# ChristianFeldmann/libHM

Measured on AMD Instinct MI355X. Metric: decoded Mpixels/s (luma), 2160p Main10 reconstruction + loop filters, higher is better.
Workload: dtype int16 samples / int32 accumulate; 1 GPU; 3840x2160 Main10 lowdelay_P pictures, pre-parsed CTU metadata: prep+MC+dequant/IT/recon+deblock+SAO, batch of 16 independent pictures per step, inputs resident in HBM; sub_benchmark=full, streams=2, parallelism=frame-parallel, 1 process per GPU, no data-path collective

## Files before the change

### libhm_amd/csrc/hmgpu_api.hip

```cpp
#include "hmgpu_host.h"

#include <algorithm>
#include <cstdio>
#include <cstring>
#include <cstdlib>
#include <new>
#include <vector>

namespace hmgpu_host __attribute__((visibility("hidden"))) {

hipError_t h2d_small(hmgpu_ctx* c, void* dst, const void* src, size_t bytes, hipStream_t hs) {
  const size_t need = (bytes + 63) & ~(size_t)63;
  if (!c->bounce || need > hmgpu_ctx::kBounceSeg) return hipMemcpyAsync(dst, src, bytes, hipMemcpyHostToDevice, hs);
  if (c->bounce_off + need > hmgpu_ctx::kBounceSeg) {
    hipStream_t streams[3] = {c->stream, c->copy_stream, c->copy_stream2};
    for (int k = 0; k < 3; k++) (void)hipEventRecord(c->bounce_ev[c->bounce_seg][k], streams[k]);
    c->bounce_used[c->bounce_seg] = true;
    c->bounce_seg = (c->bounce_seg + 1) % hmgpu_ctx::kBounceSegs;
    c->bounce_off = 0;
    if (c->bounce_used[c->bounce_seg]) for (int k = 0; k < 3; k++) (void)hipEventSynchronize(c->bounce_ev[c->bounce_seg][k]);
  }
  char* at = c->bounce + (size_t)c->bounce_seg * hmgpu_ctx::kBounceSeg + c->bounce_off;
  memcpy(at, src, bytes);
  c->bounce_off += need;
// ... 217 lines not shown

namespace hmgpu_host __attribute__((visibility("hidden"))) {

hmgpu_status run_recon(hmgpu_ctx* c, const Batch& b, bool any_intra, bool any_wp, bool any_cells, bool any_bi, bool any_islice) {
  int max_ctus = 0;
  for (int i = 0; i < b.n; i++) max_ctus = std::max(max_ctus, b.num_ctus[i]);
  { ProfScope ps(c, K_PREP); launch_prep(c->d_pics, b, max_ctus, c->parts, any_intra, any_bi, any_cells || c->fmt != 1, c->fmt, c->stream); }
  if (c->fmt != 1) {
    for (int i = 0; i < b.n; i++) {
      const PicDev& d = c->pics[b.pic[i]].dev;
      HIP_TRY(c, hipMemsetAsync(d.resid[1], 0, (size_t)((char*)d.resid[2] - (char*)d.resid[1]) + c->coef_elems[2] * sizeof(int16_t), c->stream));
    }
  }
  McArgs ma;
  memset(&ma, 0, sizeof(ma));
  ma.n = b.n; ma.width = c->seq.width; ma.height = c->seq.height; ma.log2ctu = c->seq.log2_ctu_size; ma.ctus_w = c->ctus_w;
  ma.tw = c->grid_w / 2; ma.npics = c->seq.max_pictures;
  ma.slab = c->plane_slab; ma.pic_stride = 2 * c->plane_bytes; ma.slab_bytes = ma.pic_stride * c->pics.size(); ma.sao_off = (uint32_t)c->plane_bytes;
  for (size_t i = 0; i < c->pics.size(); i++)
    if (c->pics[i].sao_applied) (i < 32 ? ma.sao_mask_lo : ma.sao_mask_hi) |= 1u << (i & 31);
  for (int i = 0; i < b.n; i++) {
    const PicDev& d = c->pics[b.pic[i]].dev;
    ma.first_ctu[i] = b.first_ctu[i]; ma.num_ctus[i] = b.num_ctus[i];
    ma.tmv[i] = d.tmv; ma.slices[i] = d.slices;
  }
  const PicDev& d0 = c->pics[b.pic[0]].dev;
  const char* const base0 = (const char*)c->pics[b.pic[0]].planes;
  uint32_t bps = (uint32_t)std::max(4, std::min(b.n >= 4 ? 12 : 24, max_ctus / 8 + 1));
  {
    ItxArgs ia;
    memset(&ia, 0, sizeof(ia));
    ia.n = b.n; ia.class_mask = 0xf;
    for (int k = 0; k < 3; k++) { ia.rtw[k] = (c->grid_w / 2) >> (k ? c->csx : 0); ia.bd[k] = d0.bd[k]; }
    ia.csx = c->csx; ia.csy = c->csy;
    for (int k = 0; k < 4; k++) ia.tu_cap[k] = c->tu_cap[k];
    for (int i = 0; i < b.n; i++) {
      const PicDev& d = c->pics[b.pic[i]].dev;
      for (int k = 0; k < 4; k++) ia.tu[i][k] = d.tu[k];
      ia.tu_count[i] = d.tu_count;
      for (int k = 0; k < 3; k++) { ia.coef[i][k] = d.coef[k]; ia.resid[i][k] = d.resid[k]; }
      ia.sl_m[i] = d.sl_m;
    }
    ProfScope ps(c, K_ITX);
    launch_itx(ia, bps, c->stream);
    bool any_ccp = false;
    for (int i = 0; i < b.n; i++) any_ccp |= c->pics[b.pic[i]].dev.ccp[0] != nullptr;
    if (any_ccp) launch_ccp(c->d_pics, b, max_ctus, c->stream);
  }
  {
    ProfScope ps(c, K_MC_LUMA);
    ma.pitch = c->pitch[0]; ma.bd = c->seq.bit_depth_luma;
    ma.origin_off = (uint32_t)((const char*)d0.rec[0] - base0);
    ma.rtw = c->grid_w / 2;
    for (int i = 0; i < b.n; i++) { ma.dst[i] = c->pics[b.pic[i]].dev.rec[0]; ma.resid[i] = c->pics[b.pic[i]].dev.resid[0]; }
    launch_mc_luma(ma, max_ctus, any_wp, any_bi, c->stream);
    if (any_cells) { ProfScope pc(c, K_MC_CELLS); launch_mc_luma_cells(c->d_pics, c->d_finals, b, max_ctus, c->seq.log2_ctu_size, any_wp, c->stream); }
  }
  if (c->fmt != 1) {
    ProfScope ps(c, K_MC_CHROMA);
    launch_mc_chroma_fmt(c->d_pics, c->d_finals, b, max_ctus, c->seq.log2_ctu_size, c->fmt, any_wp, c->stream);
  } else if (c->seq.chroma_format != 0) {
    ProfScope ps(c, K_MC_CHROMA);
    ma.pitch = c->pitch[1]; ma.bd = c->seq.bit_depth_chroma;
    ma.origin_off = (uint32_t)((const char*)d0.rec[1] - base0);
    ma.cr_off = 0;
    ma.rtw = c->grid_w / 4;
    for (int i = 0; i < b.n; i++) {
      const PicDev& d = c->pics[b.pic[i]].dev;
      ma.dst[i] = d.rec[1]; ma.dst2[i] = d.rec[2]; ma.resid[i] = d.resid[1]; ma.resid2[i] = d.resid[2];
    }
    launch_mc_chroma(ma, max_ctus, any_wp, any_bi, c->stream);
    if (any_cells) { ProfScope pc(c, K_MC_CELLS); launch_mc_chroma_cells(c->d_pics, c->d_finals, b, max_ctus, c->seq.log2_ctu_size, any_wp, c->stream); }
  }
  if (any_intra) {
    ProfScope ps(c, K_INTRA);
    launch_intra(c->d_pics, b, c->d_ctu_order, c->num_ctus, !any_islice, c->stream);
    if (c->fmt == 2) launch_intra_chroma_422(c->d_pics, b, c->stream);
    for (int i = 0; i < b.n; i++) if (std::find(c->intra_launched.begin(), c->intra_launched.end(), b.pic[i]) == c->intra_launched.end()) c->intra_launched.push_back(b.pic[i]);
  }
  HIP_TRY(c, hipGetLastError());
  return HMGPU_OK;
}

hmgpu_status run_filter(hmgpu_ctx* c, const Batch& b, int stages) {
  bool all_sao = stages == 7 && c->fmt == 1;
  for (int i = 0; i < b.n && all_sao; i++) all_sao = c->pics[b.pic[i]].sao_any;
  if (all_sao) {
    bool nofilt = false;
    for (int i = 0; i < b.n; i++) nofilt |= c->pics[b.pic[i]].dev.any_nofilt != 0;
    { ProfScope ps(c, K_FILTER); launch_filter_fused(c->d_pics, b, c->seq.width, c->seq.height, nofilt, c->stream); }
    HIP_TRY(c, hipGetLastError());
    return HMGPU_OK;
  }
  if (stages & 1) { ProfScope ps(c, K_DBK_VER); launch_deblock(c->d_pics, b, 0, c->seq.width, c->seq.height, c->stream);
                    if (c->fmt != 1) launch_deblock_chroma_fmt(c->d_pics, b, 0, c->seq.width, c->seq.height, c->stream); }
  if (stages & 2) { ProfScope ps(c, K_DBK_HOR); launch_deblock(c->d_pics, b, 1, c->seq.width, c->seq.height, c->stream);
                    if (c->fmt != 1) launch_deblock_chroma_fmt(c->d_pics, b, 1, c->seq.width, c->seq.height, c->stream); }
  if (stages & 4) {
    bool any = false;
    for (int i = 0; i < b.n; i++) any |= c->pics[b.pic[i]].sao_any;
    if (any) { ProfScope ps(c, K_SAO); launch_sao(c->d_pics, b, c->seq.width, c->seq.height, c->csx, c->csy, c->stream); }
  }
  HIP_TRY(c, hipGetLastError());
  return HMGPU_OK;
}

hmgpu_status stage_sao(hmgpu_ctx* c, Picture& p, const hmgpu_pic_params* pp, const hmgpu_sao_param* sao,
                       const std::vector<uint16_t>& slice_idx, const std::vector<uint16_t>& tile_idx) {
  const int n = c->num_ctus;
  std::vector<const hmgpu_sao_param*> res((size_t)n * 3);
  std::vector<SaoDev>& dev = p.h_saoprm;
  dev.resize((size_t)n * 3);
  bool any = false;
  for (int a = 0; a < n; a++) {
    const int cx = a % c->ctus_w, cy = a / c->ctus_w;
    const hmgpu_sao_param* const* merge[2] = {nullptr, nullptr};
    auto same = [&](int o) { return slice_idx[o] == slice_idx[a] && tile_idx[o] == tile_idx[a]; };
    if (cx > 0 && same(a - 1)) merge[HMGPU_SAO_MERGE_LEFT] = &res[(size_t)(a - 1) * 3];
    if (cy > 0 && same(a - c->ctus_w)) merge[HMGPU_SAO_MERGE_ABOVE] = &res[(size_t)(a - c->ctus_w) * 3];
    unsigned avail = 1u << 4;
    for (int k = 0; k < 9; k++) {
      if (k == 4) continue;
      const int nx = cx + k % 3 - 1, ny = cy + k / 3 - 1;
      if (nx < 0 || nx >= c->ctus_w || ny < 0 || ny >= c->ctus_h) continue;
      const int o = ny * c->ctus_w + nx;
      bool ok = true;
      if (slice_idx[o] != slice_idx[a]) {
        const SliceDev& later = p.slices[std::max(slice_idx[o], slice_idx[a])];
        ok = later.lf_across_slices != 0;
      }
      if (ok && !pp->lf_across_tiles) ok = tile_idx[o] == tile_idx[a];
      if (ok) avail |= 1u << k;
    }
    for (int comp = 0; comp < 3; comp++) {
      const hmgpu_sao_param* r = &sao[(size_t)a * 3 + comp];
      if (r->mode_idc == HMGPU_SAO_MERGE) {
        if (r->type_idc < 0 || r->type_idc > 1 || !merge[r->type_idc]) return HMGPU_EINVAL;
        r = merge[r->type_idc][comp];
      }
      res[(size_t)a * 3 + comp] = r;
      const int shift = comp == 0 ? pp->sao_offset_shift_luma : pp->sao_offset_shift_chroma;
      SaoDev& d = dev[(size_t)a * 3 + comp];
      memset(&d, 0, sizeof(d));
      d.type = r->mode_idc == HMGPU_SAO_OFF ? -1 : (int8_t)r->type_idc;
      d.avail = (uint16_t)avail;
      if (d.type == HMGPU_SAO_BO) {
        d.band = (uint8_t)(r->type_aux_info & 31);
        for (int i = 0; i < 4; i++) d.off[i] = (int8_t)(r->offset[(r->type_aux_info + i) & 31] * (1 << shift));
      } else if (d.type >= 0) {
        for (int i = 0; i < 5; i++) d.off[i] = (int8_t)(r->offset[i] * (1 << shift));
      }
      any |= d.type >= 0;
    }
  }
  p.sao_any = any;
  HIP_TRY(c, h2d_small(c, p.dev.saoprm, dev.data(), dev.size() * sizeof(SaoDev), c->stream));
  return HMGPU_OK;
}

}

extern "C" {

const char* hmgpu_status_string(hmgpu_status s) {
  switch (s) {
    case HMGPU_OK: return "ok";
    case HMGPU_EINVAL: return "invalid argument";
    case HMGPU_EDEVICE: return "device (HIP) error";
    case HMGPU_EUNSUPPORTED: return "coding tool not supported";
    case HMGPU_ENOMEM: return "out of memory";
  }
  return "?";
}
const char* hmgpu_kernel_name(int32_t k) { return (k >= 0 && k < HMGPU_NUM_KERNELS) ? kKernelNames[k] : ""; }
// ... 283 lines not shown
  if (p.sao_applied) return HMGPU_EINVAL;
  coverage_clear(p);
  p.extended = true;
  return HMGPU_OK;
}

hmgpu_status hmgpu_picture_transfer(hmgpu_ctx* src, hmgpu_pic src_pic, hmgpu_ctx* dst, hmgpu_pic dst_pic) {
  if (!src || !dst || !valid_pic(src, src_pic) || !valid_pic(dst, dst_pic) || (src == dst && src_pic == dst_pic)) return HMGPU_EINVAL;
  const hmgpu_seq_params &a = src->seq, &b = dst->seq;
  if (a.width != b.width || a.height != b.height || a.log2_ctu_size != b.log2_ctu_size || a.bit_depth_luma != b.bit_depth_luma ||
      a.bit_depth_chroma != b.bit_depth_chroma) return HMGPU_EINVAL;
  void *from = nullptr, *to = nullptr;
  int64_t n_from = 0, n_to = 0;
  hmgpu_status st = hmgpu_picture_device_region(src, src_pic, HMGPU_REGION_FINISHED, &from, &n_from);
  if (st == HMGPU_OK) st = hmgpu_picture_device_region(dst, dst_pic, HMGPU_REGION_RECEIVE, &to, &n_to);
  if (st != HMGPU_OK) return st;
  if (n_from != n_to) return HMGPU_EINVAL;
  if (src->device != dst->device) {
    int can = 0;
    if (hipDeviceCanAccessPeer(&can, dst->device, src->device) == hipSuccess && can) {
      hipSetDevice(dst->device);
      const hipError_t e = hipDeviceEnablePeerAccess(src->device, 0);
      if (e != hipSuccess && e != hipErrorPeerAccessAlreadyEnabled) return HMGPU_EDEVICE;
      (void)hipGetLastError();
    }
  }
  hipSetDevice(src->device);
  if (!src->xfer_ev[0]) for (int k = 0; k < 2; k++) HIP_TRY(src, hipEventCreateWithFlags(&src->xfer_ev[k], hipEventDisableTiming));
  HIP_TRY(src, hipEventRecord(src->xfer_ev[0], src->stream));
  hipSetDevice(dst->device);
  HIP_TRY(dst, hipStreamWaitEvent(dst->stream, src->xfer_ev[0], 0));
  HIP_TRY(dst, hipMemcpyPeerAsync(to, dst->device, from, src->device, (size_t)n_from, dst->stream));
  HIP_TRY(dst, hipEventRecord(src->xfer_ev[1], dst->stream));
  hipSetDevice(src->device);
  HIP_TRY(src, hipStreamWaitEvent(src->stream, src->xfer_ev[1], 0));
  src->xfer_bytes += (uint64_t)n_from;
  touch(src, src_pic); commit_use(src);
  touch(dst, dst_pic); commit_use(dst);
  return hmgpu_picture_commit_received(dst, dst_pic);
}
uint64_t hmgpu_transfer_bytes(const hmgpu_ctx* c) { return c ? c->xfer_bytes : 0; }

void* hmgpu_stream(hmgpu_ctx* c) { return c ? (void*)c->stream : nullptr; }

hmgpu_status hmgpu_replay_batch(hmgpu_ctx* c, const hmgpu_pic* pics, int32_t n, int32_t stages, int32_t iters) {
  if (!c || !pics || n < 1 || n > kMaxBatch || iters < 0) return HMGPU_EINVAL;
  size_t ncalls = 0;
  for (int i = 0; i < n; i++) {
    if (!valid_pic(c, pics[i])) return HMGPU_EINVAL;
    if (i == 0) ncalls = c->pics[pics[i]].calls.size();
    else if (c->pics[pics[i]].calls.size() != ncalls) return HMGPU_EINVAL;
  }
  if ((stages & 8) && ncalls == 0) return HMGPU_EINVAL;
  hipSetDevice(c->device);
  const int lanes = (c->replay_streams == 2 && n >= 2 && !c->profiling) ? 2 : 1;
  hipStream_t const main_stream = c->stream;
  if (lanes == 2) {
    HIP_TRY(c, hipEventRecord(c->lane_ev[0], main_stream));
    HIP_TRY(c, hipStreamWaitEvent(c->stream2, c->lane_ev[0], 0));
  }
  hmgpu_status result = HMGPU_OK;
  for (int it = 0; it < iters && result == HMGPU_OK; it++) {
    for (int lane = 0; lane < lanes && result == HMGPU_OK; lane++) {
      const int lo = lanes == 2 ? (lane == 0 ? 0 : n / 2) : 0, hi = lanes == 2 ? (lane == 0 ? n / 2 : n) : n;
      c->stream = lane == 0 ? main_stream : c->stream2;
      if (stages & 8) {
        for (size_t k = 0; k < ncalls && result == HMGPU_OK; k++) {
          Batch b; memset(&b, 0, sizeof(b));
          b.n = hi - lo;
          bool any_intra = false, any_wp = false, any_cells = false, any_bi = false, any_islice = false;
          for (int i = lo; i < hi; i++) {
            const SliceCall& sc = c->pics[pics[i]].calls[k];
            b.pic[i - lo] = pics[i]; b.first_ctu[i - lo] = sc.first_ctu; b.num_ctus[i - lo] = sc.num_ctus;
            any_intra |= sc.intra; any_wp |= sc.wp; any_cells |= sc.cells; any_bi |= sc.bi; any_islice |= sc.islice;
          }
          result = ensure_refs_extended(c, b, k);
          if (result == HMGPU_OK) result = run_recon(c, b, any_intra, any_wp, any_cells, any_bi, any_islice);
        }
      }
      if ((stages & 7) && result == HMGPU_OK) {
        Batch b; memset(&b, 0, sizeof(b));
        b.n = hi - lo;
        for (int i = lo; i < hi; i++) { b.pic[i - lo] = pics[i]; b.first_ctu[i - lo] = 0; b.num_ctus[i - lo] = c->num_ctus; }
        result = run_filter(c, b, stages & 7);
        if (result == HMGPU_OK) {
          { ProfScope ps(c, K_EXTEND); launch_extend(c->d_pics, b, c->seq.width, c->seq.height, c->mx[0], c->my[0], c->csx, c->csy, c->stream); }
          if (hipGetLastError() != hipSuccess) result = HMGPU_EDEVICE;
        }
      }
    }
  }
  c->stream = main_stream;
  if (lanes == 2) {
    HIP_TRY(c, hipEventRecord(c->lane_ev[1], c->stream2));
    HIP_TRY(c, hipStreamWaitEvent(main_stream, c->lane_ev[1], 0));
  }
  for (int i = 0; i < n; i++) touch(c, pics[i]);
  commit_use(c);
  return result;
}

hmgpu_status hmgpu_set_streams(hmgpu_ctx* c, int32_t n) {
  if (!c || n < 1 || n > 2) return HMGPU_EINVAL;
  c->replay_streams = n;
  return HMGPU_OK;
}

hmgpu_status hmgpu_replay(hmgpu_ctx* c, hmgpu_pic cur, int32_t stages, int32_t iters) { return hmgpu_replay_batch(c, &cur, 1, stages, iters); }

hmgpu_status hmgpu_set_profiling(hmgpu_ctx* c, int32_t enable) {
  if (!c) return HMGPU_EINVAL;
  HIP_TRY(c, hipStreamSynchronize(c->stream));
  prof_drain(c);
  c->profiling = enable != 0;
  return HMGPU_OK;
}

hmgpu_status hmgpu_get_stats(hmgpu_ctx* c, hmgpu_stats* out, int32_t reset) {
  if (!c || !out) return HMGPU_EINVAL;
  HIP_TRY(c, hipStreamSynchronize(c->stream));
  prof_drain(c);
  memset(out, 0, sizeof(*out));
  for (int k = 0; k < HMGPU_NUM_KERNELS; k++) { out->kernel_ms[k] = c->kernel_ms[k]; out->kernel_launches[k] = c->kernel_launches[k]; }
  for (Picture& p : c->pics) {
    if (!p.in_use) continue;
    unsigned long long st[2 * kTuShards];
    HIP_TRY(c, hipMemcpy(st, p.dev.stats, sizeof(st), hipMemcpyDeviceToHost));
    for (int s = 0; s < kTuShards; s++) { out->intra_partitions += st[s]; out->inter_partitions += st[kTuShards + s]; }
    if (reset) HIP_TRY(c, hipMemset(p.dev.stats, 0, sizeof(st)));
  }
  if (reset) for (int k = 0; k < HMGPU_NUM_KERNELS; k++) { c->kernel_ms[k] = 0; c->kernel_launches[k] = 0; }
  return HMGPU_OK;
}

hmgpu_status hmgpu_inverse_transform_batch(hmgpu_ctx* c, int32_t log2_size, int32_t bit_depth, int32_t n, const int16_t* levels,
                                           const int8_t* qp_per, const int8_t* qp_rem, const uint8_t* flags, int16_t* resid) {
  if (!c || log2_size < 2 || log2_size > 5 || n < 1 || !levels || !qp_per || !qp_rem || !flags || !resid) return HMGPU_EINVAL;
  if (bit_depth < 8 || bit_depth > 12) return HMGPU_EUNSUPPORTED;
  hipSetDevice(c->device);
  const size_t elems = (size_t)n << (2 * log2_size);
  int16_t *d_lev = nullptr, *d_res = nullptr; int8_t *d_per = nullptr, *d_rem = nullptr; uint8_t* d_fl = nullptr;
  hmgpu_status st = HMGPU_OK;
  auto fail = [&](hipError_t e) { if (e != hipSuccess && st == HMGPU_OK) { c->last_err = (int32_t)e; st = HMGPU_EDEVICE; } };
  fail(hipMalloc((void**)&d_lev, elems * 2)); fail(hipMalloc((void**)&d_res, elems * 2));
  fail(hipMalloc((void**)&d_per, n)); fail(hipMalloc((void**)&d_rem, n)); fail(hipMalloc((void**)&d_fl, n));
  if (st == HMGPU_OK) {
    fail(hipMemcpy(d_lev, levels, elems * 2, hipMemcpyHostToDevice));
    fail(hipMemcpy(d_per, qp_per, n, hipMemcpyHostToDevice)); fail(hipMemcpy(d_rem, qp_rem, n, hipMemcpyHostToDevice));
    fail(hipMemcpy(d_fl, flags, n, hipMemcpyHostToDevice));
  }
  if (st == HMGPU_OK) {
    launch_itx_flat(log2_size, bit_depth, n, d_lev, d_per, d_rem, d_fl, d_res, c->stream);
    fail(hipGetLastError());
    fail(hipStreamSynchronize(c->stream));
    fail(hipMemcpy(resid, d_res, elems * 2, hipMemcpyDeviceToHost));
  }
  hipFree(d_lev); hipFree(d_res); hipFree(d_per); hipFree(d_rem); hipFree(d_fl);
  return st;
}

hmgpu_status hmgpu_mc_batch(hmgpu_ctx* c, int32_t is_chroma, int32_t bit_depth, const int16_t* ref_plane, int32_t ref_stride,
                            int32_t ref_w, int32_t ref_h, int32_t n, const int32_t* blocks, int32_t bi, int16_t* dst) {
  if (!c || !ref_plane || !blocks || !dst || n < 1 || ref_w < 1 || ref_h < 1 || ref_stride < ref_w) return HMGPU_EINVAL;
  if (bit_depth < 8 || bit_depth > 12) return HMGPU_EUNSUPPORTED;
  hipSetDevice(c->device);
  std::vector<int32_t> off(n);
  size_t total = 0;
  for (int i = 0; i < n; i++) {
// ... 40 lines not shown
```

### libhm_amd/csrc/hmgpu_host.h

```cpp
#pragma once
#include "hmgpu_dev.h"

#include <atomic>
#include <chrono>
#include <cstring>
#include <unordered_map>
#include <vector>

namespace hmgpu_host __attribute__((visibility("hidden"))) {
using namespace hmgpu;

enum { K_PREP = 0, K_MC_LUMA, K_MC_CHROMA, K_ITX, K_DBK_VER, K_DBK_HOR, K_SAO, K_EXTEND, K_H2D, K_INTRA, K_FILTER, K_UNPACK, K_MC_CELLS };

struct SliceCall { int first_ctu, num_ctus, slice_idx; bool intra, wp, cells, bi, islice, dir; };

struct Picture {
  bool in_use = false;
  bool sao_applied = false;
  bool filter_ready = false;
  bool sao_any = false;
  bool extended = false;
  std::vector<SliceCall> calls;
  void* planes = nullptr;
  void* meta = nullptr;
// ... 107 lines not shown
    }
  };
  ColourSlot colour_slot[HMGPU_COLOUR_MAX_LUTS];
  uint64_t xfer_bytes = 0;
  uint32_t* dl_fault = nullptr;
  std::vector<int> touched;
  std::vector<int> intra_launched;
  void* scratch = nullptr;
  size_t scratch_bytes = 0;
  hipEvent_t lane_ev[2] = {nullptr, nullptr};
  int replay_streams = 1;
  int32_t last_err = 0;
  int ctu = 64, pw = 16, parts = 256, ctus_w = 0, ctus_h = 0, num_ctus = 0;
  int fmt = 1, csx = 1, csy = 1;
  int pitch[3] = {0, 0, 0}, rows[3] = {0, 0, 0};
  int mx[3] = {0, 0, 0}, my[3] = {0, 0, 0};
  int grid_w = 0, grid_h = 0;
  uint32_t tu_cap[4] = {0, 0, 0, 0};
  size_t coef_elems[3] = {0, 0, 0};
  std::vector<Picture> pics;
  PicDev* d_pics = nullptr;
  PlaneSet* d_finals = nullptr;
  char* plane_slab = nullptr;
  size_t plane_bytes = 0;
  int32_t* d_ctu_order = nullptr;
  std::vector<PlaneSet> h_finals;
  bool profiling = false;
  std::vector<EventPair> pending;
  std::vector<EventPair> free_events;
  double kernel_ms[HMGPU_NUM_KERNELS] = {0};
  uint64_t kernel_launches[HMGPU_NUM_KERNELS] = {0};
};

namespace hmgpu_host __attribute__((visibility("hidden"))) {

struct HostTimer {
  hmgpu_ctx* c; int slot; std::chrono::steady_clock::time_point t0;
  HostTimer(hmgpu_ctx* c_, int slot_) : c(c_), slot(slot_) { if (c->host_timing) t0 = std::chrono::steady_clock::now(); }
  ~HostTimer() { if (c->host_timing) c->host_s[slot] += std::chrono::duration<double>(std::chrono::steady_clock::now() - t0).count(); }
};

#define HIP_TRY(ctx, expr)                                   \
  do {                                                       \
    hipError_t e__ = (expr);                                 \
    if (e__ != hipSuccess) {                                 \
      (ctx)->last_err = (int32_t)e__;                        \
      return HMGPU_EDEVICE;                                  \
    }                                                        \
  } while (0)

hipError_t h2d_small(hmgpu_ctx* c, void* dst, const void* src, size_t bytes, hipStream_t hs);

size_t align_up(size_t v, size_t a);

struct Carver {
  char* base; size_t off = 0;
  explicit Carver(void* b) : base((char*)b) {}
  template <typename T> T* take(size_t n) { T* p = base ? (T*)(base + off) : nullptr; off += align_up(n * sizeof(T), 256); return p; }
};

void* ctx_scratch(hmgpu_ctx* c, size_t bytes);
hmgpu_status check_faults(hmgpu_ctx* c);
void touch(hmgpu_ctx* c, int pic);
void commit_use(hmgpu_ctx* c);

void prof_begin(hmgpu_ctx* c, int kind, EventPair* ep);
void prof_end(hmgpu_ctx* c, EventPair* ep);
void prof_drain(hmgpu_ctx* c);
struct ProfScope {
  hmgpu_ctx* c; EventPair ep;
  ProfScope(hmgpu_ctx* ctx, int kind) : c(ctx) { prof_begin(c, kind, &ep); }
  ~ProfScope() { prof_end(c, &ep); if (c->pending.size() > 8192) prof_drain(c); }
};

void carve_meta(Carver& m, PicDev& d, size_t np, int num_ctus, size_t* grp = nullptr);
hmgpu_status push_picdev(hmgpu_ctx* c, int pic);
hmgpu_status push_final(hmgpu_ctx* c, int pic, hipStream_t hs);
bool valid_pic(const hmgpu_ctx* c, hmgpu_pic pic);
void coverage_clear(Picture& p);
void coverage_add(const hmgpu_ctx* c, Picture& p, int first_ctu, int num_ctus);
hmgpu_status ensure_extended(hmgpu_ctx* c, int pic);

hmgpu_status run_recon(hmgpu_ctx* c, const Batch& b, bool any_intra, bool any_wp, bool any_cells, bool any_bi, bool any_islice);
hmgpu_status run_filter(hmgpu_ctx* c, const Batch& b, int stages);
hmgpu_status stage_sao(hmgpu_ctx* c, Picture& p, const hmgpu_pic_params* pp, const hmgpu_sao_param* sao,
                       const std::vector<uint16_t>& slice_idx, const std::vector<uint16_t>& tile_idx);

}
```

### libhm_amd/csrc/hmgpu_input.hip

```cpp
#include "hmgpu_host.h"
#include "packed_format.h"

#include <algorithm>
#include <cstring>
#include <iterator>
#include <new>
#include <thread>
#include <vector>

static void mark_use(hmgpu_ctx* c, const Batch& b) {
  for (int i = 0; i < b.n; i++) touch(c, b.pic[i]);
  commit_use(c);
}

extern "C" {

static hmgpu_status register_slice(hmgpu_ctx* c, hmgpu_pic cur, int32_t slice_idx, const hmgpu_slice_params* sl, hipStream_t hs) {
  if (slice_idx < 0 || slice_idx >= HMGPU_MAX_SLICES || !sl) return HMGPU_EINVAL;
  if (sl->weighted_pred && (sl->wp_log2_denom[0] < 0 || sl->wp_log2_denom[0] > 7 || sl->wp_log2_denom[1] < 0 || sl->wp_log2_denom[1] > 7)) return HMGPU_EINVAL;
  Picture& p = c->pics[cur];
  for (int l = 0; l < 2; l++) {
    if (sl->num_ref_idx[l] < 0 || sl->num_ref_idx[l] > HMGPU_MAX_REF) return HMGPU_EINVAL;
    for (int i = 0; i < sl->num_ref_idx[l]; i++) if (!valid_pic(c, sl->ref_pic[l][i]) || sl->ref_pic[l][i] == cur) return HMGPU_EINVAL;
  }
// ... 505 lines not shown
        auto one = [&, i] { vs[i] = packed::validate(&c->seq, jobs[i].blob, jobs[i].bytes, &sums[i], true); };
        try { th.emplace_back(one); } catch (...) { one(); }
      }
      vs[0] = packed::validate(&c->seq, jobs[0].blob, jobs[0].bytes, &sums[0], true);
      for (std::thread& t : th) t.join();
      for (int i = 0; i < n; i++) if (vs[i] != HMGPU_OK) return vs[i];
    }
    for (int i = 0; i < n; i++) {
      const hmgpu_packed_job& j = jobs[i];
      const packed::Summary& sm = sums[i];
      if (sm.max_slice >= (uint32_t)j.num_slices) return HMGPU_EINVAL;
      if (sm.any_pcm && (!j.pcm_sample[0] || !j.pcm_sample[1] || !j.pcm_sample[2] || !((sm.groups >> packed::G_INTRA) & 1))) return HMGPU_EINVAL;
      if (sm.any_pcm && (c->seq.pcm_bit_depth_luma < 1 || c->seq.pcm_bit_depth_luma > c->seq.bit_depth_luma ||
                         c->seq.pcm_bit_depth_chroma < 1 || c->seq.pcm_bit_depth_chroma > c->seq.bit_depth_chroma)) return HMGPU_EINVAL;
    }
    return HMGPU_OK;
  };
  auto stage = [&](int i, const std::vector<int>& slices, bool wp, hipStream_t hs, SliceCall* call) {
    const hmgpu_status st = stage_packed(c, jobs[i], sums[i], slices, wp, hs, call);
    if (st == HMGPU_OK) { ua.pic[i] = jobs[i].pic; ua.blob[i] = (const char*)c->pics[jobs[i].pic].blob; }
    return st;
  };
  auto copied = [&] {
    if (c->copy_seq > 8 && hipEventQuery(c->copy_ev[(c->copy_seq - 7) % 8]) == hipSuccess)
      for (auto it = c->packed_reads.begin(); it != c->packed_reads.end();) it = it->second <= c->copy_seq - 7 ? c->packed_reads.erase(it) : std::next(it);
    for (int i = 0; i < n; i++) c->packed_reads[jobs[i].blob] = c->copy_seq;
  };
  auto expand = [&]() -> hmgpu_status {
    { ProfScope ps(c, K_UNPACK); launch_unpack_input(c->d_pics, ua, c->num_ctus, c->stream); }
    HIP_TRY(c, hipGetLastError());
    return HMGPU_OK;
  };
  return decompress_batch(c, n, jobs, check, stage, copied, expand);
}

hmgpu_status hmgpu_packed_wait(hmgpu_ctx* c, const void* blob) {
  if (!c || !blob) return HMGPU_EINVAL;
  const auto it = c->packed_reads.find(blob);
  if (it == c->packed_reads.end()) return HMGPU_OK;
  hipSetDevice(c->device);
  const uint64_t seq = c->copy_seq - it->second < 8 ? it->second : c->copy_seq;
  if (hipEventSynchronize(c->copy_ev[seq % 8]) != hipSuccess) return HMGPU_EDEVICE;
  return HMGPU_OK;
}

static hmgpu_status stage_sao_of(hmgpu_ctx* c, Picture& p, const hmgpu_pic_params* pp, const hmgpu_sao_param* sao) {
  std::vector<uint16_t> sidx = p.h_slice_idx, tidx = p.h_tile_idx;
  sidx.resize(c->num_ctus, 0);
  tidx.resize(c->num_ctus, 0);
  return stage_sao(c, p, pp, sao, sidx, tidx);
}

static hmgpu_status sao_became_picture(hmgpu_ctx* c, hmgpu_pic pic) {
  Picture& p = c->pics[pic];
  p.sao_applied = true; p.dev.sao_applied = 1;
  hmgpu_status st = push_final(c, pic, c->stream);
  if (st == HMGPU_OK) st = push_picdev(c, pic);
  return st;
}

hmgpu_status hmgpu_filter_pictures(hmgpu_ctx* c, int32_t n, const hmgpu_filter_job* jobs) {
  if (!c || !jobs || n < 1 || n > kMaxBatch) return HMGPU_EINVAL;
  for (int i = 0; i < n; i++) {
    if (!valid_pic(c, jobs[i].pic) || !jobs[i].pp) return HMGPU_EINVAL;
    if (jobs[i].pp->sao_enabled && !jobs[i].sao) return HMGPU_EINVAL;
    for (int k = 0; k < i; k++) if (jobs[k].pic == jobs[i].pic) return HMGPU_EINVAL;
  }
  hipSetDevice(c->device);
  Batch b; memset(&b, 0, sizeof(b));
  b.n = n;
  { HostTimer tsao(c, 4);
  for (int i = 0; i < n; i++) {
    Picture& p = c->pics[jobs[i].pic];
    p.sao_any = false;
    if (jobs[i].pp->sao_enabled) {
      hmgpu_status st = stage_sao_of(c, p, jobs[i].pp, jobs[i].sao);
      if (st != HMGPU_OK) return st;
    }
    p.filter_ready = true;
    b.pic[i] = jobs[i].pic; b.first_ctu[i] = 0; b.num_ctus[i] = c->num_ctus;
  }
  }
  HostTimer tf(c, 5);
  hmgpu_status st = run_filter(c, b, 7);
  if (st != HMGPU_OK) return st;
  for (int i = 0; i < n && st == HMGPU_OK; i++) {
    Picture& p = c->pics[jobs[i].pic];
    if (p.sao_any) st = sao_became_picture(c, jobs[i].pic);
    p.extended = true;
  }
  if (st != HMGPU_OK) return st;
  { ProfScope ps(c, K_EXTEND); launch_extend(c->d_pics, b, c->seq.width, c->seq.height, c->mx[0], c->my[0], c->csx, c->csy, c->stream); }
  HIP_TRY(c, hipGetLastError());
  mark_use(c, b);
  return HMGPU_OK;
}

hmgpu_status hmgpu_filter_picture_stages(hmgpu_ctx* c, hmgpu_pic cur, const hmgpu_pic_params* pp, const hmgpu_sao_param* sao,
                                         int32_t stages) {
  if (!c || !valid_pic(c, cur) || !pp) return HMGPU_EINVAL;
  if ((stages & 4) && pp->sao_enabled && !sao) return HMGPU_EINVAL;
  hipSetDevice(c->device);
  Picture& p = c->pics[cur];
  p.sao_any = false;
  if ((stages & 4) && pp->sao_enabled) {
    hmgpu_status st = stage_sao_of(c, p, pp, sao);
    if (st != HMGPU_OK) return st;
  }
  p.filter_ready = true;
  Batch b; memset(&b, 0, sizeof(b));
  b.n = 1; b.pic[0] = cur; b.first_ctu[0] = 0; b.num_ctus[0] = c->num_ctus;
  hmgpu_status st = run_filter(c, b, stages);
  if (st != HMGPU_OK) return st;
  if ((stages & 4) && p.sao_any) {
    st = sao_became_picture(c, cur);
    if (st != HMGPU_OK) return st;
  }
  p.extended = false;
  st = ensure_extended(c, cur);
  commit_use(c);
  return st;
}

hmgpu_status hmgpu_filter_picture(hmgpu_ctx* c, hmgpu_pic cur, const hmgpu_pic_params* pp, const hmgpu_sao_param* sao) {
  return hmgpu_filter_picture_stages(c, cur, pp, sao, 7);
}

}
```

### libhm_amd/csrc/k_filter.hip

```cpp
#include "hmgpu_dev.h"
#include "filter_core.h"
#include <type_traits>

namespace hmgpu {

namespace {
constexpr int kTW = 64, kTH = 64;
constexpr int kYC = kTW + 16, kYH = kTH + 8;
constexpr int kCC = kTW / 2 + 16, kCH = kTH / 2 + 4;
constexpr int kYW = kYC + 8, kCW = kCC + 8;

constexpr int kUnits = 9 * 18;
struct FilterLds {
  __attribute__((aligned(16))) int16_t y[kYH][kYW];
  __attribute__((aligned(16))) int16_t c[2][kCH][kCW];
  uint32_t unit[2][3][64];
  int32_t units[2][4];
};

struct SliceLf { int tc_off, beta_off, cb_off, cr_off; };
struct FPic {
  static constexpr int csx = 1, csy = 1;
  int width, height, bd0, bd1, bd2, log2ctu, ctus_w, pitch[2], grid_w, any_nofilt, mono;
  __device__ inline int bd(int comp) const { return comp == 0 ? bd0 : comp == 1 ? bd1 : bd2; }
  const int16_t* rec[2];
  int16_t* sao[2];
  const uint16_t* slice_idx;
  const SliceDev* slices;
  const BlkInfo* blk;
  const EdgeRec* edges;
  const SaoDev* saoprm;
  SliceLf s0;
};
template <typename T> __device__ inline T ldc(const T* p) { return *(const T __attribute__((address_space(4)))*)p; }
__device__ inline FPic pic_state(const PicDev* p) {
  FPic f;
  f.width = ldc(&p->width); f.height = ldc(&p->height);
  f.bd0 = ldc(&p->bd[0]); f.bd1 = ldc(&p->bd[1]); f.bd2 = ldc(&p->bd[2]);
  f.log2ctu = ldc(&p->log2ctu); f.ctus_w = ldc(&p->ctus_w);
  f.pitch[0] = ldc(&p->pitch[0]); f.pitch[1] = ldc(&p->pitch[1]);
  f.grid_w = ldc(&p->grid_w);
  f.rec[0] = ldc(&p->rec[0]); f.rec[1] = ldc(&p->rec[1]);
  f.sao[0] = ldc(&p->sao[0]); f.sao[1] = ldc(&p->sao[1]);
  f.any_nofilt = ldc(&p->any_nofilt); f.mono = ldc(&p->mono);
  f.slice_idx = ldc(&p->slice_idx); f.slices = ldc(&p->slices);
  f.blk = ldc(&p->blk); f.edges = ldc(&p->edges); f.saoprm = ldc(&p->saoprm);
  const SliceDev* s = f.slices;
  f.s0 = {ldc(&s->tc_offset_div2), ldc(&s->beta_offset_div2), ldc(&s->pps_cb_qp_offset), ldc(&s->pps_cr_qp_offset)};
  return f;
}

struct Span {
  __amdgpu_buffer_rsrc_t rs;
  uint32_t bytes;
  __device__ inline Span(const void* base, uint32_t n) : rs(__builtin_amdgcn_make_buffer_rsrc(const_cast<void*>(base), 0, n, 0x00020000)), bytes(n) {}
  __device__ inline uint32_t at(bool valid, uint32_t off) const { return valid ? off : bytes; }
  __device__ inline u32x4 load4(uint32_t off) const { return __builtin_bit_cast(u32x4, __builtin_amdgcn_raw_buffer_load_b128(rs, off, 0, 0)); }
  __device__ inline uint32_t load_u16(uint32_t off) const { return (uint16_t)__builtin_amdgcn_raw_buffer_load_b16(rs, off, 0, 0); }
  __device__ inline void store4(uint32_t off, u32x4 v) const { __builtin_amdgcn_raw_buffer_store_b128(__builtin_bit_cast(decltype(__builtin_amdgcn_raw_buffer_load_b128(rs, 0, 0, 0)), v), rs, off, 0, 0); }
};

struct SaoPrm { uint32_t w0, off_lo, off_hi; };
__device__ inline SaoPrm sao_fetch(const Span& sp, uint32_t off) {
  const auto v = __builtin_amdgcn_raw_buffer_load_b96(sp.rs, off, 0, 0);
  return {(uint32_t)v[0], (uint32_t)v[1], (uint32_t)v[2]};
}

template <int W, bool NF>
__device__ inline u32x4 sao_group(const FPic& P, int comp, const int16_t (*t)[W], int ox, int oy, int x, int row, const SaoPrm& prm) {
  const int cs = comp ? 1 : 0;
  const int w = P.width >> cs, h = P.height >> cs;
  const int log2ctb = P.log2ctu - cs;
  const int cx = x >> log2ctb, cy = row >> log2ctb;
  const uint32_t w0 = prm.w0;
  const int type = (int)(int8_t)(w0 & 0xff);
  const int16_t* line = &t[row - oy][x - ox];
  const u32x4 cur = *reinterpret_cast<const u32x4*>(line);
  if (type < 0) return cur;
  const uint32_t off_lo = prm.off_lo, off_hi = prm.off_hi;
  const int bd = P.bd(comp), maxv = (1 << bd) - 1;
  uint32_t out[4];
  if (type == HMGPU_SAO_BO) {
    const int shift = bd - 5, band0 = (w0 >> 8) & 0xff;
    const uint32_t c[4] = {cur.x, cur.y, cur.z, cur.w};
#pragma unroll
    for (int j = 0; j < 4; j++) {
      const uint32_t lo = c[j] & 0xffffu, hi = c[j] >> 16;
      const uint32_t k0 = min(((lo >> shift) - band0) & 31u, 4u), k1 = min(((hi >> shift) - band0) & 31u, 4u);
      const s16x2 off = lut_offsets(k0 | (k1 << 16), off_lo, 0u);
      out[j] = as_u32(__builtin_elementwise_min(__builtin_elementwise_max(as_s16x2(c[j]) + off, splat(0)), splat(maxv)));
    }
  } else {
    const int ctb = 1 << log2ctb;
    const int x0 = cx << log2ctb, y0 = cy << log2ctb;
    const int x1 = min(x0 + ctb, w) - 1, y1 = min(y0 + ctb, h) - 1;
    const unsigned av = w0 >> 16;
    auto run = [&](auto dxc, auto dyc) {
      constexpr int DX = decltype(dxc)::value, DY = decltype(dyc)::value;
      const int16_t* ra = line + DY * W;
      const int16_t* rb = line - DY * W;
      const u32x4 ea = *reinterpret_cast<const u32x4*>(ra), eb = *reinterpret_cast<const u32x4*>(rb);
      uint32_t na[4], nb[4];
      uint32_t la = 0, raa = 0, lb = 0, rbb = 0;
      if constexpr (DX < 0) { la = (uint16_t)ra[-1]; rbb = (uint16_t)rb[8]; }
      if constexpr (DX > 0) { raa = (uint16_t)ra[8]; lb = (uint16_t)rb[-1]; }
      shifted<DX>(ea, la, raa, na);
      shifted<-DX>(eb, lb, rbb, nb);
      sao_eo_core<DX, DY>(x, row, cur, na, nb, off_lo, off_hi, av, x0, y0, x1, y1, maxv, out);
    };
    switch (type) {
      case HMGPU_SAO_EO_0:   run(std::integral_constant<int, -1>{}, std::integral_constant<int, 0>{}); break;
      case HMGPU_SAO_EO_90:  run(std::integral_constant<int, 0>{}, std::integral_constant<int, -1>{}); break;
      case HMGPU_SAO_EO_135: run(std::integral_constant<int, -1>{}, std::integral_constant<int, -1>{}); break;
      default:               run(std::integral_constant<int, 1>{}, std::integral_constant<int, -1>{}); break;
    }
  }
  if (NF && P.any_nofilt) {
    uint32_t m[4];
    sao_exempt_mask(P, comp, x, row, m);
    const uint32_t c[4] = {cur.x, cur.y, cur.z, cur.w};
#pragma unroll
    for (int j = 0; j < 4; j++) out[j] = (c[j] & m[j]) | (out[j] & ~m[j]);
  }
// ... 5 lines not shown
}
static_assert(HMGPU_MAX_SLICES <= 4096, "slice index must fit the 12 bits of a list entry");

template <bool NF>
__device__ inline uint32_t edge_classify(uint32_t rec, uint32_t slice, int u) {
  const uint32_t bs = rec & 3u, qp = (rec >> 2) & 127u;
  const uint32_t p_nf = NF ? (rec >> 9) & 1u : 0u, q_nf = NF ? (rec >> 10) & 1u : 0u;
  const uint32_t e = (uint32_t)u | (bs << 8) | (p_nf << 10) | (q_nf << 11) | ((qp + 32u) << 12) | (slice << 20);
  return bs ? e : 0u;
}

__device__ inline void push_units(uint32_t (&list)[3][64], int32_t (&count)[4], uint32_t rec, int t) {
  const unsigned long long m = __ballot(rec != 0u);
  const int wave = t >> 6, lane = t & 63;
  if (rec != 0u) list[wave][__popcll(m & ((1ull << lane) - 1ull))] = rec;
  if (lane == 0) count[wave] = __popcll(m);
}
__device__ inline uint32_t pop_unit(const uint32_t (&list)[3][64], const int32_t (&count)[4], int t) {
  const int c0 = count[0], c1 = count[1], c2 = count[2];
  if (t < c0) return list[0][t];
  if (t < c0 + c1) return list[1][t - c0];
  if (t < c0 + c1 + c2) return list[2][t - c0 - c1];
  return 0u;
}

template <int DIR, bool NF>
__device__ inline void edge_apply(const FPic& P, FilterLds& L, int x0, int y0, uint32_t rec) {
  if (rec == 0u) return;
  const int u = rec & 0xff, bs = (rec >> 8) & 3, qp = (int)((rec >> 12) & 0xff) - 64, slice = rec >> 20;
  const bool p_nf = NF && ((rec >> 10) & 1), q_nf = NF && ((rec >> 11) & 1);
  const int x = DIR == 0 ? x0 + 8 * (u % 9) : x0 - 4 + 4 * (u % 18);
  const int y = DIR == 0 ? y0 - 4 + 4 * (u / 9) : y0 + 8 * (u / 18);
  const SliceLf sl = slice == 0 ? P.s0 : slice_lf(P.slices + slice);
  const int tc_off = sl.tc_off, beta_off = sl.beta_off;
  int16_t* base = &L.y[y - (y0 - 4)][x - (x0 - 8)];
  uint32_t a[8], b[8];
  if (DIR == 0) {
    uint32_t r[4][4];
#pragma unroll
    for (int i = 0; i < 4; i++) {
      const u32x2 lo = *reinterpret_cast<const u32x2*>(base + i * kYW - 4), hi = *reinterpret_cast<const u32x2*>(base + i * kYW);
      r[i][0] = lo.x; r[i][1] = lo.y; r[i][2] = hi.x; r[i][3] = hi.y;
    }
    rows_to_pairs(r[0], r[1], a);
    rows_to_pairs(r[2], r[3], b);
  } else {
#pragma unroll
    for (int k = 0; k < 8; k++) {
      const u32x2 v = *reinterpret_cast<const u32x2*>(base + (k - 4) * kYW);
      a[k] = v.x; b[k] = v.y;
    }
  }
  filter_luma_unit(a, b, bs, qp, tc_off, beta_off, P.bd(0), p_nf, q_nf);
  if (DIR == 0) {
    uint32_t r[4][4];
    pairs_to_rows(a, r[0], r[1]);
    pairs_to_rows(b, r[2], r[3]);
#pragma unroll
    for (int i = 0; i < 4; i++) {
      *reinterpret_cast<u32x2*>(base + i * kYW - 4) = (u32x2){r[i][0], r[i][1]};
      *reinterpret_cast<u32x2*>(base + i * kYW) = (u32x2){r[i][2], r[i][3]};
    }
  } else {
#pragma unroll
    for (int k = 1; k < 7; k++) *reinterpret_cast<u32x2*>(base + (k - 4) * kYW) = (u32x2){a[k], b[k]};
  }
  if (bs == 2 && ((DIR == 0 ? x : y) & 15) == 0 && !P.mono) {
    const int maxc = (1 << P.bd(1)) - 1;
#pragma unroll
    for (int comp = 1; comp < 3; comp++) {
      const int tc = chroma_tc(qp, comp == 1 ? sl.cb_off : sl.cr_off, tc_off, P.bd(comp));
      int16_t* cb = &L.c[comp - 1][(y >> 1) - ((y0 >> 1) - 2)][(x >> 1) - ((x0 >> 1) - 8)];
#pragma unroll
      for (int i = 0; i < 2; i++) {
        int16_t* s = DIR == 0 ? cb + i * kCW : cb + i;
        const int o = DIR == 0 ? 1 : kCW;
        const int m2 = (uint16_t)s[-2 * o], m3 = (uint16_t)s[-o], m4 = (uint16_t)s[0], m5 = (uint16_t)s[o];
        const int delta = clip3(-tc, tc, ((((m4 - m3) << 2) + m2 - m5 + 4) >> 3));
        if (!p_nf) s[-o] = (int16_t)clip3(0, maxc, m3 + delta);
        if (!q_nf) s[0] = (int16_t)clip3(0, maxc, m4 - delta);
      }
    }
  }
}

}

template <bool NF>
__global__ void __launch_bounds__(256) k_filter_fused(const PicDev* __restrict__ pics, Batch b, int tiles_x, int tiles) {
  __shared__ FilterLds L;
  int slot, lb;
  if (!xcd_remap(blockIdx.x, b.n, tiles, slot, lb)) return;
  const FPic P = pic_state(pics + b.pic[slot]);
  __builtin_amdgcn_sched_barrier(0);
  const int x0 = (lb % tiles_x) * kTW, y0 = (lb / tiles_x) * kTH;
  const int t = threadIdx.x;
  const int l2 = P.log2ctu, p0 = P.pitch[0], p1 = P.pitch[1];
  const int vx = x0 + 8 * (t % 9), vy = y0 - 4 + 4 * (t / 9), hx = x0 - 4 + 4 * (t % 18), hy = y0 + 8 * (t / 18);
  const bool vin = t < kUnits && vy >= 0 && vx < P.width && vy < P.height, hin = t < kUnits && hx >= 0 && hx < P.width && hy < P.height;
  const int ecw = P.grid_w >> 1, ex0 = (x0 >> 3) - 1, ey0 = (y0 >> 3) - 1;
  const Span se(reinterpret_cast<const char*>(P.edges) + ((ptrdiff_t)ey0 * ecw + ex0) * (ptrdiff_t)sizeof(EdgeRec), (uint32_t)((9 * ecw + 10) * (int)sizeof(EdgeRec)));
  const uint32_t ev = se.load_u16(se.at(vin, (uint32_t)((((vy >> 3) - ey0) * ecw + (vx >> 3) - ex0) * 8 + ((vy >> 2) & 1) * 2)));
  const uint32_t eh = se.load_u16(se.at(hin, (uint32_t)((((hy >> 3) - ey0) * ecw + (hx >> 3) - ex0) * 8 + 4 + ((hx >> 2) & 1) * 2)));
  const int sx0 = (x0 - 8) >> l2, sy0 = (y0 - 8) >> l2;
  const Span ss(reinterpret_cast<const char*>(P.slice_idx) + ((ptrdiff_t)sy0 * P.ctus_w + sx0) * 2,
                P.slice_idx ? (uint32_t)(((((y0 + 64) >> l2) - sy0) * P.ctus_w + ((x0 + 64) >> l2) - sx0 + 1) * 2) : 0u);
  uint32_t sv = ss.load_u16(ss.at(vin, (uint32_t)((((vy >> l2) - sy0) * P.ctus_w + (vx >> l2) - sx0) * 2)));
  uint32_t sh = ss.load_u16(ss.at(hin, (uint32_t)((((hy >> l2) - sy0) * P.ctus_w + (hx >> l2) - sx0) * 2)));
  constexpr int VPR = kYC / 8, VPC = 2 * kCC / 8;
  static_assert(kYH * VPR > 512 && kYH * VPR <= 768 && kCH * VPC > 256 && kCH * VPC <= 512, "three rounds of luma vectors, two of chroma");
  const int yr0 = t / VPR, yv0 = t % VPR, yr1 = (t + 256) / VPR, yv1 = (t + 256) % VPR, yr2 = (t + 512) / VPR, yv2 = (t + 512) % VPR;
  const int ur0 = t / VPC, uv0 = t % VPC, ur1 = (t + 256) / VPC, uv1 = (t + 256) % VPC;
  const bool yin2 = t + 512 < kYH * VPR, uin1 = t + 256 < kCH * VPC;
  const Span sy(P.rec[0] + ((ptrdiff_t)(y0 - 4) * p0 + (x0 - 8)), (uint32_t)(((kYH - 1) * p0 + kYC) * 2));
  const Span sc(P.rec[1] + ((ptrdiff_t)((y0 >> 1) - 2) * p1 + kCStep * ((x0 >> 1) - 8)), (uint32_t)(((kCH - 1) * p1 + kCStep * kCC) * 2));
  const u32x4 ty0 = sy.load4((uint32_t)((yr0 * p0 + 8 * yv0) * 2));
  const u32x4 ty1 = sy.load4((uint32_t)((yr1 * p0 + 8 * yv1) * 2));
  const u32x4 ty2 = sy.load4(sy.at(yin2, (uint32_t)((yr2 * p0 + 8 * yv2) * 2)));
  const u32x4 tc0 = sc.load4((uint32_t)((ur0 * p1 + 8 * uv0) * 2));
  const u32x4 tc1 = sc.load4(sc.at(uin1, (uint32_t)((ur1 * p1 + 8 * uv1) * 2)));
  const int gx = (t & 7) * 8, gy = t >> 3;
  const int lx = x0 + gx, ly[2] = {y0 + gy, y0 + gy + 32};
  const int ccomp = 1 + (t & 1), ccx = (x0 >> 1) + ((t >> 1) & 3) * 8, ccy = (y0 >> 1) + gy;
  const bool lin[2] = {lx < P.width && ly[0] < P.height, lx < P.width && ly[1] < P.height}, cin = ccx < (P.width >> 1) && ccy < (P.height >> 1);
  const int n64 = 63 >> l2;
  const Span sp(P.saoprm + ((ptrdiff_t)(y0 >> l2) * P.ctus_w + (x0 >> l2)) * 3, (uint32_t)(((n64 * P.ctus_w + n64) * 3 + 3) * (int)sizeof(SaoDev)));
  const uint32_t prow = (uint32_t)(3 * (int)sizeof(SaoDev)) * (uint32_t)P.ctus_w;
  const SaoPrm sl0 = sao_fetch(sp, sp.at(lin[0], (uint32_t)(gy >> l2) * prow + (uint32_t)((gx >> l2) * 3 * (int)sizeof(SaoDev))));
  const SaoPrm sl1 = sao_fetch(sp, sp.at(lin[1], (uint32_t)((gy + 32) >> l2) * prow + (uint32_t)((gx >> l2) * 3 * (int)sizeof(SaoDev))));
  const SaoPrm sc0 = sao_fetch(sp, sp.at(cin, (uint32_t)((2 * gy) >> l2) * prow + (uint32_t)(((((t >> 1) & 3) * 16) >> l2) * 3 + ccomp) * (uint32_t)sizeof(SaoDev)));
  asm volatile("" : "+v"(sv), "+v"(sh));
  if (t < 192) {
    push_units(L.unit[0], L.units[0], edge_classify<NF>(ev, sv, t), t);
    push_units(L.unit[1], L.units[1], edge_classify<NF>(eh, sh, t), t);
  }
  *reinterpret_cast<u32x4*>(&L.y[yr0][8 * yv0]) = ty0;
  *reinterpret_cast<u32x4*>(&L.y[yr1][8 * yv1]) = ty1;
  if (yin2) *reinterpret_cast<u32x4*>(&L.y[yr2][8 * yv2]) = ty2;
  auto put_chroma = [&](int r, int v, const u32x4 c) {
    *reinterpret_cast<u32x2*>(&L.c[0][r][4 * v]) = u32x2{__builtin_amdgcn_perm(c.y, c.x, 0x05040100u), __builtin_amdgcn_perm(c.w, c.z, 0x05040100u)};
    *reinterpret_cast<u32x2*>(&L.c[1][r][4 * v]) = u32x2{__builtin_amdgcn_perm(c.y, c.x, 0x07060302u), __builtin_amdgcn_perm(c.w, c.z, 0x07060302u)};
  };
  put_chroma(ur0, uv0, tc0);
  if (uin1) put_chroma(ur1, uv1, tc1);
  __syncthreads();
  edge_apply<0, NF>(P, L, x0, y0, pop_unit(L.unit[0], L.units[0], t));
  __syncthreads();
  edge_apply<1, NF>(P, L, x0, y0, pop_unit(L.unit[1], L.units[1], t));
  __syncthreads();
  const Span oy(P.sao[0] + ((ptrdiff_t)y0 * p0 + x0), (uint32_t)(((kTH - 1) * p0 + kTW) * 2));
  if (lin[0]) oy.store4((uint32_t)((gy * p0 + gx) * 2), sao_group<kYW, NF>(P, 0, L.y, x0 - 8, y0 - 4, lx, ly[0], sl0));
  if (lin[1]) oy.store4((uint32_t)(((gy + 32) * p0 + gx) * 2), sao_group<kYW, NF>(P, 0, L.y, x0 - 8, y0 - 4, lx, ly[1], sl1));
  if (cin) {
    const u32x4 own = sao_group<kCW, NF>(P, ccomp, L.c[ccomp - 1], (x0 >> 1) - 8, (y0 >> 1) - 2, ccx, ccy, sc0);
    const bool odd = t & 1;
    const uint32_t r0 = (uint32_t)__shfl_xor((int)(odd ? own.x : own.z), 1, 64), r1 = (uint32_t)__shfl_xor((int)(odd ? own.y : own.w), 1, 64);
    const uint32_t cb0 = odd ? r0 : own.x, cb1 = odd ? r1 : own.y, cr0 = odd ? own.z : r0, cr1 = odd ? own.w : r1;
    const u32x4 o = {__builtin_amdgcn_perm(cr0, cb0, 0x05040100u), __builtin_amdgcn_perm(cr0, cb0, 0x07060302u),
                     __builtin_amdgcn_perm(cr1, cb1, 0x05040100u), __builtin_amdgcn_perm(cr1, cb1, 0x07060302u)};
    const Span oc(P.sao[1] + ((ptrdiff_t)(y0 >> 1) * p1 + kCStep * (x0 >> 1)), (uint32_t)(((kTH / 2 - 1) * p1 + kCStep * kTW / 2) * 2));
    oc.store4((uint32_t)((gy * p1 + kCStep * (((t >> 1) & 3) * 8 + (odd ? 4 : 0))) * 2), o);
  }
}

void launch_filter_fused(const PicDev* pics, const Batch& b, int width, int height, bool nofilt, hipStream_t s) {
  const int tiles_x = (width + kTW - 1) / kTW, tiles = tiles_x * ((height + kTH - 1) / kTH);
  dim3 grid((unsigned)xcd_grid(b.n, tiles));
  if (nofilt) hipLaunchKernelGGL(k_filter_fused<true>, grid, dim3(256), 0, s, pics, b, tiles_x, tiles);
  else hipLaunchKernelGGL(k_filter_fused<false>, grid, dim3(256), 0, s, pics, b, tiles_x, tiles);
}

}
```

Baseline: 188,500 Mpixels/s.

## Fuse reference-picture border extension into the fused filter kernel

```diff
diff --git a/libhm_amd/csrc/hmgpu_api.hip b/libhm_amd/csrc/hmgpu_api.hip
--- a/libhm_amd/csrc/hmgpu_api.hip
+++ b/libhm_amd/csrc/hmgpu_api.hip
@@ -323,7 +323,8 @@
   return HMGPU_OK;
 }
 
-hmgpu_status run_filter(hmgpu_ctx* c, const Batch& b, int stages) {
+hmgpu_status run_filter(hmgpu_ctx* c, const Batch& b, int stages, bool* fused) {
+  *fused = false;
   bool all_sao = stages == 7 && c->fmt == 1;
   for (int i = 0; i < b.n && all_sao; i++) all_sao = c->pics[b.pic[i]].sao_any;
   if (all_sao) {
@@ -331,6 +332,8 @@
     for (int i = 0; i < b.n; i++) nofilt |= c->pics[b.pic[i]].dev.any_nofilt != 0;
     { ProfScope ps(c, K_FILTER); launch_filter_fused(c->d_pics, b, c->seq.width, c->seq.height, nofilt, c->stream); }
     HIP_TRY(c, hipGetLastError());
+    for (int i = 0; i < b.n; i++) c->pics[b.pic[i]].extended = true;
+    *fused = true;
     return HMGPU_OK;
   }
   if (stages & 1) { ProfScope ps(c, K_DBK_VER); launch_deblock(c->d_pics, b, 0, c->seq.width, c->seq.height, c->stream);
@@ -780,8 +783,9 @@
         Batch b; memset(&b, 0, sizeof(b));
         b.n = hi - lo;
         for (int i = lo; i < hi; i++) { b.pic[i - lo] = pics[i]; b.first_ctu[i - lo] = 0; b.num_ctus[i - lo] = c->num_ctus; }
-        result = run_filter(c, b, stages & 7);
-        if (result == HMGPU_OK) {
+        bool fused = false;
+        result = run_filter(c, b, stages & 7, &fused);
+        if (result == HMGPU_OK && !fused) {
           { ProfScope ps(c, K_EXTEND); launch_extend(c->d_pics, b, c->seq.width, c->seq.height, c->mx[0], c->my[0], c->csx, c->csy, c->stream); }
           if (hipGetLastError() != hipSuccess) result = HMGPU_EDEVICE;
         }
diff --git a/libhm_amd/csrc/hmgpu_host.h b/libhm_amd/csrc/hmgpu_host.h
--- a/libhm_amd/csrc/hmgpu_host.h
+++ b/libhm_amd/csrc/hmgpu_host.h
@@ -213,7 +213,7 @@
 hmgpu_status ensure_extended(hmgpu_ctx* c, int pic);
 
 hmgpu_status run_recon(hmgpu_ctx* c, const Batch& b, bool any_intra, bool any_wp, bool any_cells, bool any_bi, bool any_islice);
-hmgpu_status run_filter(hmgpu_ctx* c, const Batch& b, int stages);
+hmgpu_status run_filter(hmgpu_ctx* c, const Batch& b, int stages, bool* fused);
 hmgpu_status stage_sao(hmgpu_ctx* c, Picture& p, const hmgpu_pic_params* pp, const hmgpu_sao_param* sao,
                        const std::vector<uint16_t>& slice_idx, const std::vector<uint16_t>& tile_idx);
 
diff --git a/libhm_amd/csrc/hmgpu_input.hip b/libhm_amd/csrc/hmgpu_input.hip
--- a/libhm_amd/csrc/hmgpu_input.hip
+++ b/libhm_amd/csrc/hmgpu_input.hip
@@ -611,7 +611,8 @@
   }
   }
   HostTimer tf(c, 5);
-  hmgpu_status st = run_filter(c, b, 7);
+  bool fused = false;
+  hmgpu_status st = run_filter(c, b, 7, &fused);
   if (st != HMGPU_OK) return st;
   for (int i = 0; i < n && st == HMGPU_OK; i++) {
     Picture& p = c->pics[jobs[i].pic];
@@ -619,8 +620,10 @@
     p.extended = true;
   }
   if (st != HMGPU_OK) return st;
-  { ProfScope ps(c, K_EXTEND); launch_extend(c->d_pics, b, c->seq.width, c->seq.height, c->mx[0], c->my[0], c->csx, c->csy, c->stream); }
-  HIP_TRY(c, hipGetLastError());
+  if (!fused) {
+    { ProfScope ps(c, K_EXTEND); launch_extend(c->d_pics, b, c->seq.width, c->seq.height, c->mx[0], c->my[0], c->csx, c->csy, c->stream); }
+    HIP_TRY(c, hipGetLastError());
+  }
   mark_use(c, b);
   return HMGPU_OK;
 }
@@ -639,13 +642,14 @@
   p.filter_ready = true;
   Batch b; memset(&b, 0, sizeof(b));
   b.n = 1; b.pic[0] = cur; b.first_ctu[0] = 0; b.num_ctus[0] = c->num_ctus;
-  hmgpu_status st = run_filter(c, b, stages);
+  bool fused = false;
+  hmgpu_status st = run_filter(c, b, stages, &fused);
   if (st != HMGPU_OK) return st;
   if ((stages & 4) && p.sao_any) {
     st = sao_became_picture(c, cur);
     if (st != HMGPU_OK) return st;
   }
-  p.extended = false;
+  if (!fused) p.extended = false;
   st = ensure_extended(c, cur);
   commit_use(c);
   return st;
diff --git a/libhm_amd/csrc/k_filter.hip b/libhm_amd/csrc/k_filter.hip
--- a/libhm_amd/csrc/k_filter.hip
+++ b/libhm_amd/csrc/k_filter.hip
@@ -21,7 +21,7 @@
 struct SliceLf { int tc_off, beta_off, cb_off, cr_off; };
 struct FPic {
   static constexpr int csx = 1, csy = 1;
-  int width, height, bd0, bd1, bd2, log2ctu, ctus_w, pitch[2], grid_w, any_nofilt, mono;
+  int width, height, bd0, bd1, bd2, log2ctu, ctus_w, pitch[2], mx, my, grid_w, any_nofilt, mono;
   __device__ inline int bd(int comp) const { return comp == 0 ? bd0 : comp == 1 ? bd1 : bd2; }
   const int16_t* rec[2];
   int16_t* sao[2];
@@ -39,6 +39,7 @@
   f.bd0 = ldc(&p->bd[0]); f.bd1 = ldc(&p->bd[1]); f.bd2 = ldc(&p->bd[2]);
   f.log2ctu = ldc(&p->log2ctu); f.ctus_w = ldc(&p->ctus_w);
   f.pitch[0] = ldc(&p->pitch[0]); f.pitch[1] = ldc(&p->pitch[1]);
+  f.mx = ldc(&p->mx[0]); f.my = ldc(&p->my[0]);
   f.grid_w = ldc(&p->grid_w);
   f.rec[0] = ldc(&p->rec[0]); f.rec[1] = ldc(&p->rec[1]);
   f.sao[0] = ldc(&p->sao[0]); f.sao[1] = ldc(&p->sao[1]);
@@ -210,6 +211,36 @@
       }
     }
   }
+}
+
+template <int E>
+__device__ inline void put_margins(const int16_t* out, int opitch, int16_t* org, int pitch, int vw, int vh, bool el, bool er, bool et, bool eb,
+                                   int mx, int my, int t) {
+  constexpr int VE = 8 / E;
+  const int xl = el ? mx : 0, yt = et ? my : 0;
+  const int rows = yt + vh + (eb ? my : 0);
+  const Span sm(org - ((ptrdiff_t)yt * pitch + E * xl), (uint32_t)(((rows - 1) * pitch + E * (xl + vw + (er ? mx : 0))) * 2));
+  const int nl = xl / VE, ns = nl + (er ? mx / VE : 0);
+  for (int r = t >> 4; r < rows; r += 16) {
+    const int16_t* line = out + clip3(0, vh - 1, r - yt) * opitch;
+    for (int k = t & 15; k < ns; k += 16) {
+      const bool right = k >= nl;
+      const int16_t* e = line + E * (right ? vw - 1 : 0);
+      uint32_t v;
+      if constexpr (E == 1) v = (uint16_t)e[0] * 0x10001u;
+      else v = *reinterpret_cast<const uint32_t*>(e);
+      const int x = right ? xl + vw + (k - nl) * VE : k * VE;
+      sm.store4((uint32_t)((r * pitch + E * x) * 2), u32x4{v, v, v, v});
+    }
+  }
+  const int nt = yt, nb = nt + (eb ? my : 0);
+  const int k = t & 7;
+  if (k * VE < vw)
+    for (int r = t >> 3; r < nb; r += 32) {
+      const bool below = r >= nt;
+      const u32x4 v = *reinterpret_cast<const u32x4*>(out + (below ? vh - 1 : 0) * opitch + 8 * k);
+      sm.store4((uint32_t)(((below ? vh + r : r) * pitch + E * xl + 8 * k) * 2), v);
+    }
 }
 
 }
@@ -277,18 +308,38 @@
   edge_apply<1, NF>(P, L, x0, y0, pop_unit(L.unit[1], L.units[1], t));
   __syncthreads();
   const Span oy(P.sao[0] + ((ptrdiff_t)y0 * p0 + x0), (uint32_t)(((kTH - 1) * p0 + kTW) * 2));
-  if (lin[0]) oy.store4((uint32_t)((gy * p0 + gx) * 2), sao_group<kYW, NF>(P, 0, L.y, x0 - 8, y0 - 4, lx, ly[0], sl0));
-  if (lin[1]) oy.store4((uint32_t)(((gy + 32) * p0 + gx) * 2), sao_group<kYW, NF>(P, 0, L.y, x0 - 8, y0 - 4, lx, ly[1], sl1));
+  u32x4 fy0, fy1, fc;
+  asm("" : "=v"(fy0), "=v"(fy1), "=v"(fc));
+  if (lin[0]) { fy0 = sao_group<kYW, NF>(P, 0, L.y, x0 - 8, y0 - 4, lx, ly[0], sl0); oy.store4((uint32_t)((gy * p0 + gx) * 2), fy0); }
+  if (lin[1]) { fy1 = sao_group<kYW, NF>(P, 0, L.y, x0 - 8, y0 - 4, lx, ly[1], sl1); oy.store4((uint32_t)(((gy + 32) * p0 + gx) * 2), fy1); }
   if (cin) {
     const u32x4 own = sao_group<kCW, NF>(P, ccomp, L.c[ccomp - 1], (x0 >> 1) - 8, (y0 >> 1) - 2, ccx, ccy, sc0);
     const bool odd = t & 1;
     const uint32_t r0 = (uint32_t)__shfl_xor((int)(odd ? own.x : own.z), 1, 64), r1 = (uint32_t)__shfl_xor((int)(odd ? own.y : own.w), 1, 64);
     const uint32_t cb0 = odd ? r0 : own.x, cb1 = odd ? r1 : own.y, cr0 = odd ? own.z : r0, cr1 = odd ? own.w : r1;
-    const u32x4 o = {__builtin_amdgcn_perm(cr0, cb0, 0x05040100u), __builtin_amdgcn_perm(cr0, cb0, 0x07060302u),
-                     __builtin_amdgcn_perm(cr1, cb1, 0x05040100u), __builtin_amdgcn_perm(cr1, cb1, 0x07060302u)};
+    fc = u32x4{__builtin_amdgcn_perm(cr0, cb0, 0x05040100u), __builtin_amdgcn_perm(cr0, cb0, 0x07060302u),
+               __builtin_amdgcn_perm(cr1, cb1, 0x05040100u), __builtin_amdgcn_perm(cr1, cb1, 0x07060302u)};
     const Span oc(P.sao[1] + ((ptrdiff_t)(y0 >> 1) * p1 + kCStep * (x0 >> 1)), (uint32_t)(((kTH / 2 - 1) * p1 + kCStep * kTW / 2) * 2));
-    oc.store4((uint32_t)((gy * p1 + kCStep * (((t >> 1) & 3) * 8 + (odd ? 4 : 0))) * 2), o);
-  }
+    oc.store4((uint32_t)((gy * p1 + kCStep * (((t >> 1) & 3) * 8 + (odd ? 4 : 0))) * 2), fc);
+  }
+  const bool el = x0 == 0, er = x0 + kTW >= P.width, et = y0 == 0, eb = y0 + kTH >= P.height;
+  if (!(el || er || et || eb)) return;
+  constexpr int kFC = kCStep * kTW / 2;
+  static_assert(kTH <= kYH && kTW <= kYW && kTH / 2 * kFC * 2 <= (int)sizeof(L.c), "the final samples fit the copies' space");
+  int16_t* const fcs = &L.c[0][0][0];
+  int tb = t;
+  asm volatile("" : "+v"(tb));
+  const int by = tb >> 3, bx = (tb & 7) * 8;
+  const int bp = ((tb >> 1) & 3) * 8 + (tb & 1) * 4;
+  __syncthreads();
+  if (lin[0]) *reinterpret_cast<u32x4*>(&L.y[by][bx]) = fy0;
+  if (lin[1]) *reinterpret_cast<u32x4*>(&L.y[by + 32][bx]) = fy1;
+  if (cin) *reinterpret_cast<u32x4*>(fcs + by * kFC + kCStep * bp) = fc;
+  __syncthreads();
+  const int vw = min(kTW, P.width - x0), vh = min(kTH, P.height - y0);
+  put_margins<1>(&L.y[0][0], kYW, P.sao[0] + ((ptrdiff_t)y0 * p0 + x0), p0, vw, vh, el, er, et, eb, P.mx, P.my, tb);
+  if (!P.mono)
+    put_margins<kCStep>(fcs, kFC, P.sao[1] + ((ptrdiff_t)(y0 >> 1) * p1 + kCStep * (x0 >> 1)), p1, vw >> 1, vh >> 1, el, er, et, eb, P.mx >> 1, P.my >> 1, tb);
 }
 
 void launch_filter_fused(const PicDev* pics, const Batch& b, int width, int height, bool nofilt, hipStream_t s) {
```

Result: faster. 192,300 Mpixels/s (median of 6 runs) (+2.0%).
